# OpenDriveLab/ThinkTwice

Hardware: AMD Instinct MI355X
Metric: frames/sec forward (4-cam+LiDAR, thinktwice.py cfg) (higher is better)
Workload: dtype bf16x3h; 1 GPU; forward_inference thinktwice.py cfg: 8 frames x (2 sweeps x 4 cams x 448x896 + 65536-pt LiDAR), ResNet50+PAFPN+DepthNet+UNet+LSS splat, LidarNet, fusion, 5-stage decoder; parallelism=replicas x1 (no data-path collective), launch=eager launches, 3 batches in flight on alternating streams, batches_in_flight=3

## Files before the change

### include/thinktwice_hip.h

```cpp
#ifndef THINKTWICE_HIP_H
#define THINKTWICE_HIP_H

#include <stddef.h>
#include <stdint.h>

#ifdef __cplusplus
extern "C" {
#endif

#define TT_F32 0
#define TT_BF16 1
#define TT_F16 2

#define TT_ACT_NONE 0
#define TT_ACT_RELU 1
#define TT_ACT_SIGMOID 2
#define TT_ACT_GELU 3
#define TT_ACT_SOFTPLUS 4
#define TT_ACT_SOFTPLUS_CLAMP 5

const char* tt_last_error(void);
const char* tt_conv_last_kernel(void);
int tt_conv_set_trace(void* stamps_or_null);
int tt_version(void);

int tt_voxel_pool_fwd(int batch_size, int num_points, int num_channels,
                      int num_voxel_x, int num_voxel_y, int num_voxel_z,
                      const int32_t* geom_xyz, const float* input_features,
                      float* output_features, int32_t* pos_memo, void* stream);

long long tt_voxel_pool_workspace_bytes(int batch_size, int num_points, int num_channels,
                                        int num_voxel_x, int num_voxel_y);
int tt_voxel_pool_fwd_ws(int batch_size, int num_points, int num_channels,
                         int num_voxel_x, int num_voxel_y, int num_voxel_z,
                         const int32_t* geom_xyz, const float* input_features,
                         float* output_features, int32_t* pos_memo,
                         void* workspace, long long workspace_bytes, void* stream);

long long tt_voxel_pool_plan_bytes(int batch_size, int num_points, int num_voxel_x, int num_voxel_y);
long long tt_voxel_pool_plan_workspace_bytes(int batch_size, int num_points);
int tt_voxel_pool_plan_build(int batch_size, int num_points, int num_voxel_x, int num_voxel_y, int num_voxel_z,
                             const int32_t* geom_xyz, void* workspace, long long workspace_bytes, void* plan,
                             long long plan_bytes, void* stream);
long long tt_voxel_pool_planned_workspace_bytes(int batch_size, int num_points, int num_channels, int num_voxel_x,
                                                int num_voxel_y);
int tt_voxel_pool_fwd_planned(int batch_size, int num_points, int num_channels, int num_voxel_x, int num_voxel_y,
                              const void* plan, const float* input_features, float* output_features, void* workspace,
                              long long workspace_bytes, void* stream);

int tt_voxel_pool_bwd(int batch_size, int num_points, int num_channels,
                      int num_voxel_x, int num_voxel_y,
                      const int32_t* pos_memo, const float* grad_out_bhwc,
                      float* grad_in, void* stream);

int tt_frustum_voxel_index(int batch_size, int num_cams, int D, int fH, int fW,
                           const float* frustum, const float* mats,
                           const float* voxel_lo, const float* voxel_size,
                           int32_t* geom_xyz, float* geom_f32_or_null,
                           void* stream);

int tt_lift_splat_fwd(int batch_size, int num_cams, int D, int fH, int fW, int C,
                      int num_voxel_x, int num_voxel_y, int num_voxel_z,
                      const void* depth_logits, const void* context, int dtype,
                      const int32_t* geom_xyz, float* out, int out_cstride,
                      int out_coff, int rot_flip, void* stream);

long long tt_lift_splat_workspace_bytes(int batch_size, int num_cams, int D, int fH, int fW, int C,
                                        int num_voxel_x, int num_voxel_y);
int tt_lift_splat_fwd_ws(int batch_size, int num_cams, int D, int fH, int fW, int C,
                         int num_voxel_x, int num_voxel_y, int num_voxel_z,
                         const void* depth_logits, const void* context, int dtype,
                         const int32_t* geom_xyz, float* out, int out_cstride,
                         int out_coff, int rot_flip, void* ws, long long ws_bytes, void* stream);

typedef struct tt_conv_desc {
    const void* in;   int N, H, W, Cin, in_cstride, in_coff;
    long long in_nstride;
    const void* weight; int Cout, KH, KW, stride, pad, dil;
    void* out; int OH, OW, out_cstride, out_coff;
    long long out_nstride;
    int pixel_shuffle2;
    const float* scale; const float* shift;
    const float* shift_n; int shift_n_mod;
    const void* res1; int res1_cstride, res1_coff;
    const void* res2; int res2_cstride, res2_coff;
    int act;
    int dtype;
    int out_dtype;
    const int* gather_idx;
    const int* m_dev;
    float* splitk_ws;
    const void* weight_x3;
    const int* row_perm;
    const unsigned* row_mask;
    int splitk_slices;
    int in_pair, out_pair;
    const void* weight_h2;
    float* out2; int out2_cstride, out2_coff;
    int res1_up_h, res1_up_w;
    int res1_f32;
    int in_up2;
} tt_conv_desc;

int tt_conv2d_fwd(const tt_conv_desc* d, void* stream);
int tt_conv2d_splitk_slices(const tt_conv_desc* d);
int tt_conv2d_plan(const tt_conv_desc* d, char* label, int label_bytes);

int tt_seg_feedback_chain(const float* x, long long R, int x_stride, int K1, const float* w1, const float* scale1,
                          const float* shift1, int act1, const float* w2, const void* w2_x3, int N2, const float* scale2,
                          const float* shift2, int act2, float* out, int out_stride, int out_coff, void* stream);

typedef struct tt_chain_stage {
    const void* w; const float* bias;
    int K, Kp, N, act, in_sel;
    const float* res; int res_stride, res_coff;
    const float* side; const float* side_w; int side_stride, side_k;
    float* out; int out_stride, out_coff;
} tt_chain_stage;
int tt_mlp_chain(const float* x, long long R, int x_stride, int nstages, const tt_chain_stage* stages, int n_split,
                 void* stream);
long long tt_mlp_chain_wide_workspace_bytes(long long R, int nstages, const tt_chain_stage* stages);
int tt_mlp_chain_wide(const float* x, long long R, int x_stride, int nstages, const tt_chain_stage* stages, int n_groups,
                      void* workspace, long long workspace_bytes, void* stream);
int tt_mlp_chain_wide_max_workgroups(void);
int tt_mlp_chain_wide_faults(void);
int tt_device_faults(void);
int tt_clear_device_faults(void);
int tt_mlp_chain_wide_set_max_spin(int polls);
int tt_mlp_chain_wide_set_trace(void* stamps_or_null);

long long tt_dec_gru_scratch_floats(int B);
int tt_dec_gru(int B, const float* inp6, const float* state, float* fut, float* scratch, const void* const* w0,
               const float* const* wx, const float* const* b0, const void* const* w2, const float* const* b2,
               const void* wd0, const float* bd0, const void* wd2, const float* bd2, void* stream);
long long tt_dec_flatten_scratch_floats(int maps);
int tt_dec_flatten(int maps, const float* in, float* out, float* mids_or_null, float* scratch, const void* const* w,
                   const float* const* b, const float* bn_scale, const float* bn_shift, void* stream);
int tt_dec_set_trace(void* stamps_or_null);
long long tt_dec_bev_update_scratch_floats(int B);
int tt_dec_bev_update(int B, const float* bev, const float* G, float* out, long long out_bstride, float* out2,
                      long long out2_bstride, float* scratch, const void* w0, const float* b0, const void* const* w2,
                      const float* b2, void* stream);

int tt_nchw_to_nhwc_pad(const float* in, void* out, int N, int C, int H, int W, int Cp,
                        int out_dtype, void* stream);
int tt_nchw_to_nhwc_border(const float* in, void* out, int N, int C, int H, int W, int Cp, int Hp, int Wp,
                           int top, int left, int out_dtype, void* stream);
int tt_nhwc_to_nchw(const void* in, float* out, int N, int C, int H, int W, int cstride, int coff,
                    int in_dtype, void* stream);
int tt_maxpool3x3s2(const void* in, void* out, int N, int H, int W, int C, int dtype, void* stream);
int tt_upsample_nearest_add(void* dst, const void* src, int N, int H, int W, int C, int h, int w,
                            int dtype, void* stream);
int tt_bilinear_up2(const void* in, void* out, int N, int H, int W, int C, int dtype, void* stream);
int tt_bilinear_up2_pair(const float* in, float* out, int N, int H, int W, int C, void* stream);
int tt_spatial_pool(const void* in, float* out, int N, int HW, int C, int cstride, int coff, int mode,
                    int dtype, void* stream);
int tt_channel_gate(const void* x, const float* gate, const void* res, void* out, int N, int HW, int C,
                    int gate_act, int out_act, int dtype, void* stream);
int tt_affine_rows(const void* x, const float* scale, const float* shift, void* out, long long R, int C,
                   int x_stride, int out_stride, int act, int dtype, void* stream);
int tt_layernorm_rows(const void* x, const float* gamma, const float* beta, void* out, long long R,
                      int D, int x_stride, int out_stride, float eps, int dtype, void* stream);
int tt_copy_nhwc(const void* in, void* out, int N, int H, int W, int C, int in_cstride, int in_coff,
                 int out_cstride, int out_coff, int rot_flip, int in_dtype, int out_dtype, void* stream);
int tt_broadcast_rows(const void* v, void* out, int N, int HW, int C, int v_stride, int out_cstride,
                      int out_coff, int dtype, void* stream);
int tt_ew(const void* a, const void* b, const void* g, void* out, long long R, int C, int a_stride,
          int a_coff, int b_stride, int b_coff, int g_stride, int g_coff, int o_stride, int o_coff,
          int op, int act, int dtype, void* stream);
int tt_concat_rows(float* out, long long R, int out_stride, int nseg, const float* const* srcs, const int* strides,
                   const int* widths, const int* coffs, const int* divs, const int* mods, void* stream);

int tt_deform_im2col3x3(const void* x, const float* offsets, void* cols, int N, int H, int W, int C,
                        int off_cstride, int pad, int dtype, void* stream);

int tt_look_project_pack(int B, const float* wp, const float* lidar2img, const float* ida_mat,
                         float img_h, float img_w, float* ref_packed, int* query_of_slot,
                         int* count, int* max_len, void* stream);
int tt_look_gather_query(int B, const int* query_of_slot, const float* ref_packed, const float* wp,
                         const float* ctrl_softplus, const float* temporal_embedding,
                         const float* static_embedding, const float* measurement_feat,
                         const float* flattened_feat, const void* const* level_maps,
                         const int* level_hw, int maps_dtype, float* out, int row_stride, void* stream);
int tt_msda_sample(int B, const void* value, int value_dtype, const float* offsets, const float* logits,
                   const float* ref_packed, const int* level_hw, float* out, void* stream);
int tt_msda_sample_strided(int B, const void* value, int value_dtype, int value_cstride, int value_coff,
                           const float* offsets, const float* logits, const float* ref_packed, const int* level_hw,
                           float* out, void* stream);
int tt_sca_reduce(int B, const float* x, const int* max_len, float* out, void* stream);
// ... 316 lines not shown
```

### thinktwice_amd/csrc/conv_igemm.hip

```cpp
#include <stdlib.h>

#include "conv_common.h"

namespace tt {

template <typename T, int BM, int BN, int WAVES_M, int WAVES_N, bool GATHER, int KX = 1>
__global__ __launch_bounds__(256) void conv_igemm_kernel(const ConvArgs p) {
    constexpr int VEC = Elem<T>::kVec;
    constexpr int BKB = ((sizeof(T) == 4) ? 64 : 128) * KX;
    constexpr int BK = BKB / (int)sizeof(T);
    constexpr int VPR = BKB / 16;
    constexpr int ROWB = BKB + 16;
    constexpr int NVA = (BM * VPR + 255) / 256;
    constexpr int NVB = (BN * VPR + 255) / 256;
    constexpr int WTM = BM / WAVES_M, WTN = BN / WAVES_N;
    constexpr int TM = WTM / 32, TN = WTN / 32;
    static_assert(WAVES_M * WAVES_N == 4, "4 waves");

    extern __shared__ __attribute__((aligned(16))) unsigned char smem[];
    const int nbuf = (p.K > BK) ? 2 : 1;
    unsigned char* sA = smem;
    unsigned char* sB = smem + nbuf * BM * ROWB;

    const int tid = threadIdx.x;
    const int lane = tid & 63;
    const int wave = tid >> 6;
    const int wm = wave / WAVES_N, wn = wave % WAVES_N;

    const int tile_n = blockIdx.x % p.tiles_n;
    const int tile_m = blockIdx.x / p.tiles_n;
    const int m0 = tile_m * BM, n0 = tile_n * BN;
    int Mlim = p.M;
    if (p.m_dev) {
        const int md = *p.m_dev;
        Mlim = md < Mlim ? md : Mlim;
    }
    if (m0 >= Mlim) return;

    const T* __restrict__ in = reinterpret_cast<const T*>(p.in);
    const T* __restrict__ wgt = reinterpret_cast<const T*>(p.weight);

    int a_row[NVA], a_vc[NVA], a_h0[NVA], a_w0[NVA];
    long long a_base[NVA];
    bool a_ok[NVA];
#pragma unroll
    for (int i = 0; i < NVA; ++i) {
        const int idx = tid + 256 * i;
        a_row[i] = idx / VPR;
        a_vc[i] = idx % VPR;
        const int m = m0 + a_row[i];
        a_ok[i] = (m < Mlim) && (idx < BM * VPR);
        const int mm = a_ok[i] ? m : 0;
        if (GATHER) {
            a_h0[i] = 0;
            a_w0[i] = 0;
            a_base[i] = (long long)mm * (p.KH * p.KW);
        } else {
            const int n = mm / (p.OH * p.OW);
            const int r = mm - n * (p.OH * p.OW);
            const int oh = r / p.OW, ow = r - oh * p.OW;
            a_h0[i] = oh * p.stride - p.pad;
            a_w0[i] = ow * p.stride - p.pad;
            a_base[i] = (long long)n * p.in_nstride + p.in_coff;
        }
    }
    int b_row[NVB], b_vc[NVB];
    bool b_ok[NVB];
#pragma unroll
    for (int i = 0; i < NVB; ++i) {
        const int idx = tid + 256 * i;
        b_row[i] = idx / VPR;
        b_vc[i] = idx % VPR;
        b_ok[i] = ((n0 + b_row[i]) < p.Cout) && (idx < BN * VPR);
    }

    int jn[NVA];
#pragma unroll
    for (int i = 0; i < NVA; ++i) jn[i] = -1;
    const int nk_all = (p.K + BK - 1) / BK;
    int kt0 = 0, nk = nk_all;
    if (p.splits > 1) {
        const int per = (nk_all + p.splits - 1) / p.splits;
        kt0 = blockIdx.y * per;
        nk = min(nk_all, kt0 + per);
        if (kt0 >= nk) return;
// ... 290 lines not shown
    ConvChoice c;
    if (const int r = conv2d_prepare(d, a, f)) return r;
    if (const int r = conv_choose(a, f, &c)) return r;
    hipStream_t st = (hipStream_t)stream;
    const bool pair = d->in_pair || d->out_pair;
    const char* what = "tt_conv2d_fwd";
    int r;
    if (c.x3) a.weight = d->weight_x3;
    switch (c.family) {
        case CONV_H2:
        case CONV_H2_PIPE:
            a.weight = d->weight_h2;
            what = "tt_conv2d_fwd(h2)";
            r = launch_conv_h2(c, a, st);
            break;
        case CONV_SMALL:
            what = "tt_conv2d_fwd(small)";
            r = launch_conv_small(a, d->dtype, st);
            break;
        case CONV_SP_RUNS_L2:
            what = "tt_conv2d_fwd(sp l2)";
            r = launch_sp_conv_l2(c, a, st);
            break;
        case CONV_SP_RUNS:
            what = "tt_conv2d_fwd(glds x3)";
            r = launch_sp_conv_runs(c, a, st);
            break;
        case CONV_X3_PIPE:
        case CONV_X3_RUN3:
            what = pair ? "tt_conv2d_fwd(glds x3, pair)" : "tt_conv2d_fwd(glds x3)";
            r = launch_conv_x3_pipe(c, a, st);
            break;
        case CONV_X3_UP2:
            what = "tt_conv2d_fwd(x3 up2)";
            r = launch_conv_x3_up2(c, a, st);
            break;
        case CONV_X3_PATCH:
            what = "tt_conv2d_fwd(x3 patch, pair)";
            r = launch_conv_x3_patch(c, a, st);
            break;
        case CONV_GLDS:
            what = !c.x3 ? "tt_conv2d_fwd(glds)" : c.splits > 1 ? "tt_conv2d_fwd(glds x3 split-K)" : pair ? "tt_conv2d_fwd(glds x3, pair)" : "tt_conv2d_fwd(glds x3)";
            if (c.splits > 1) a.ws_slices = c.slices;
            r = launch_conv_glds(c, a, d->dtype, st);
            break;
        default:
            a.row_perm = nullptr;
            a.row_mask = nullptr;
            r = launch_conv_igemm(c, a, d->dtype, st);
            break;
    }
    if (r < 0) return r;
    conv_label(c, d->dtype, g_conv_kernel, sizeof(g_conv_kernel));
    if (c.main_rows > 0) {
        ConvArgs t = a;
        t.m_begin = c.main_rows * 256;
        if (launch_conv_glds(conv_tail_choice(c), t, d->dtype, st) < 0) return -1;
    }
    if (c.splits > 1) launch_splitk_finalize(a, d->dtype, st);
    return check_launch(what);
}

extern "C" int tt_conv2d_splitk_slices(const tt_conv_desc* d) {
    ConvArgs a;
    ConvFacts f;
    ConvChoice c;
    if (conv2d_prepare(d, a, f)) return 0;
    if (d->in_pair || d->out_pair || d->in_up2 || d->weight_h2 || d->res1_up_w > 0) return 0;
    f.assume_ws = true;
    if (conv_choose(a, f, &c)) return 0;
    return c.splits > 1 ? c.slices : 0;
}

extern "C" int tt_conv2d_plan(const tt_conv_desc* d, char* label, int label_bytes) {
    ConvArgs a;
    ConvFacts f;
    ConvChoice c;
    if (const int r = conv2d_prepare(d, a, f)) return r;
    if (const int r = conv_choose(a, f, &c)) return r;
    TT_REQUIRE(label && label_bytes > 0, "tt_conv2d_plan: no room for the label");
    conv_label(c, d->dtype, label, (size_t)label_bytes);
    return 0;
}
```

### thinktwice_amd/csrc/conv_igemm_glds.hip

```cpp
#include "conv_lds_dma.h"

namespace tt {

#ifndef TT_GLDS_DEBUG
#define TT_GLDS_DEBUG 0
#endif

template <typename T, int BN, int WAVES_M, int WAVES_N, int BKB, int STAGES = 3, bool GATHER = false, bool X3 = false, bool APAIR = false>
__global__ __launch_bounds__(WAVES_M * WAVES_N * 64,
                             ((256 / WAVES_M / 32) * (BN / WAVES_N / 32) >= 16)  ? 1
                             : ((256 / WAVES_M / 32) * (BN / WAVES_N / 32) >= 8) ? 2
                             : (WAVES_M * WAVES_N == 16 || BKB == 64)            ? 4
                                                                                 : 2)
void conv_igemm_glds_kernel(const ConvArgs p, const void* zero_page,
                                                              int tiles_m, int tiles_n) {
#if defined(__HIP_DEVICE_COMPILE__)
    constexpr int BM = 256;
    constexpr int VEC = Elem<T>::kVec;
    constexpr int BK = BKB / (int)sizeof(T);
    constexpr int CPR = BKB / 16;
    constexpr bool ASYM = STAGES == 23;
    constexpr int SA = ASYM ? 3 : STAGES, SB = ASYM ? 2 : STAGES;
    static_assert(STAGES == 2 || STAGES == 3 || ASYM, "2 or 3 LDS stages, or 23 = 3 activation + 2 weight stages");
    static_assert(!GATHER || STAGES == 2, "gather mode is written for the 2-stage pipeline");
// ... 64 lines not shown
    const T* b_ptr[NIB];
#pragma unroll
    for (int j = 0; j < NIB; ++j) {
        const int g = ((wave + NW * j) % NB_INSTR) * 64 + lane;
        const int row = g / CPR, pos = g % CPR;
        b_c[j] = (pos ^ swz<BKB>(row)) * VEC;
        b_ok[j] = (n0 + row) < p.Cout;
        b_base[j] = (long long)(n0 + row) * p.K;
        b_ptr[j] = wgt + b_base[j] + b_c[j];
    }

    int nk = (p.K + BK - 1) / BK;

    int g_cur[NIA];
    int g_t = 0;
    const int cin_shift = 31 - __clz(p.Cin), cin_mask = p.Cin - 1;
    constexpr int TPTMAX = 4;
    const bool planned = GATHER && p.row_mask != nullptr;
    unsigned umask = 0;
    if (planned) {
        unsigned* uw = reinterpret_cast<unsigned*>(smem);
        if (tid == 0) *uw = 0u;
        __syncthreads();
        if (tid < BM && m0 + tid < Mlim) atomicOr(uw, p.row_mask[m0 + tid]);
        __syncthreads();
        umask = *uw;
        __syncthreads();
        umask = __builtin_amdgcn_readfirstlane(umask);
        const int nt = __popc(umask);
        nk = p.Cin >= BK ? nt * (p.Cin / BK) : (nt * p.Cin + BK - 1) / BK;
    }
    struct TapWalk {
        unsigned rem;
        int sub, cur;
    };
    TapWalk wf{umask, 0, -1}, wi{umask, 0, -1};
    auto next_taps = [&](TapWalk& w, int (&tp)[TPTMAX]) {
        if (p.Cin >= BK) {
            if (w.sub == 0) {
                w.cur = w.rem ? __builtin_ctz(w.rem) : -1;
                w.rem &= w.rem - 1;
            }
            tp[0] = w.cur;
            if (++w.sub == p.Cin / BK) w.sub = 0;
        } else {
            const int tpt = BK >> cin_shift;
#pragma unroll
            for (int i = 0; i < TPTMAX; ++i) {
                tp[i] = -1;
                if (i < tpt && w.rem) {
                    tp[i] = __builtin_ctz(w.rem);
                    w.rem &= w.rem - 1;
                }
            }
        }
    };
    auto pick = [&](const int (&tp)[TPTMAX], int slot) {
        int t = tp[0];
#pragma unroll
        for (int i = 1; i < TPTMAX; ++i) t = (slot == i) ? tp[i] : t;
        return t;
    };
    auto fetch_rulebook = [&]() {
        if (planned) {
            int tp[TPTMAX];
            next_taps(wf, tp);
#pragma unroll
            for (int j = 0; j < NIA; ++j) {
                const int t = p.Cin >= BK ? tp[0] : pick(tp, a_c[j] >> cin_shift);
                g_cur[j] = (a_ok[j] && t >= 0) ? p.gather[a_base[j] + t] : -1;
            }
            ++g_t;
            return;
        }
#pragma unroll
        for (int j = 0; j < NIA; ++j) {
            const int k = g_t * BK + a_c[j];
            g_cur[j] = (a_ok[j] && k < p.K) ? p.gather[a_base[j] + (k >> cin_shift)] : -1;
        }
        ++g_t;
    };
    const int wave_s = __builtin_amdgcn_readfirstlane(wave);
    const unsigned lds_dma_base = (unsigned)(uintptr_t)(__attribute__((address_space(3))) unsigned char*)smem;
    KWalk wa{0, 0, 0}, wb{0, 0, 0};
    if (!GATHER && p.splits > 1) {
        const int per = (nk + p.splits - 1) / p.splits;
        const int kt0 = (int)blockIdx.y * per;
        int kt1 = kt0 + per;
        kt1 = kt1 < nk ? kt1 : nk;
        const int taps = p.KH * p.KW;
        const int chunk = kt0 / taps, tap = kt0 - chunk * taps;
        wa.ci = wb.ci = chunk * BK;
        wa.kh = wb.kh = tap / p.KW;
        wa.kw = wb.kw = tap - (tap / p.KW) * p.KW;
        nk = kt1 > kt0 ? kt1 - kt0 : 0;
    }
    auto issue_a = [&](int kt) {
        const unsigned st = lds_dma_base + (unsigned)off_a(kt);
        const int kh = wa.kh, kw = wa.kw, ci = wa.ci;
        const int k0 = kt * BK;
        const int tap = kh * p.KW + kw;
        const long long tap_off = ((long long)(kh * p.dil) * p.W + kw * p.dil) * p.in_cstride + ci;
        advance<BK>(wa, p);
        const bool dbg_skip_a = TT_GLDS_DEBUG && p.act == 98 && kt > 0;
#pragma unroll
        for (int j = 0; j < NIA; ++j) {
            if (dbg_skip_a) break;
            const T* src;
            if (GATHER) {
                const int gi = g_cur[j];
                const int kl = k0 + a_c[j];
                src = gi >= 0 ? in + (long long)gi * p.in_cstride + p.in_coff + (kl & cin_mask) : zp;
            } else {
                src = ((a_mask[j] >> tap) & 1u) ? a_ptr[j] + tap_off : zp;
            }
            dma_piece(src, st + (unsigned)(wave_s + NW * j) * 1024u);
        }
    };
    auto issue_b = [&](int kt) {
        const unsigned st = lds_dma_base + (unsigned)off_b(kt);
        const int k0 = GATHER ? kt * BK
                              : (wb.kh * p.KW + wb.kw) * p.Cin + wb.ci;
        advance<BK>(wb, p);
        const bool dbg_skip_b = TT_GLDS_DEBUG && p.act == 97 && kt > 0;
        int tpi[TPTMAX];
        if (planned) next_taps(wi, tpi);
#pragma unroll
        for (int j = 0; j < NIB; ++j) {
            if (dbg_skip_b) break;
            bool ok = b_ok[j] && (!GATHER || (k0 + b_c[j] < p.K));
            const T* src = ok ? b_ptr[j] + k0 : zp;
            if (planned) {
                const int t = p.Cin >= BK ? tpi[0] : pick(tpi, b_c[j] >> cin_shift);
                ok = b_ok[j] && t >= 0;
                src = ok ? b_ptr[j] - b_c[j] + (long long)t * p.Cin + ((k0 + b_c[j]) & cin_mask) : zp;
            }
            dma_piece(src, st + (unsigned)((wave_s + NW * j) % NB_INSTR) * 1024u);
        }
    };
    auto issue_tile = [&](int kt) {
        issue_a(kt);
        issue_b(kt);
    };
    auto issue_ahead = [&](int kt) {
        if (ASYM) {
            if (kt + 1 < nk) issue_b(kt + 1);
            if (kt + 2 < nk) issue_a(kt + 2);
        } else if (kt + STAGES - 1 < nk) {
            issue_tile(kt + STAGES - 1);
        }
    };

    auto a_begin = [&](int kt, bool on) { return dma_begin_a<BK>(p, wa, lds_dma_base + (unsigned)off_a(kt), on); };
    auto b_begin = [&](int kt, bool on) { return dma_begin_b<BK, 1>(p, wb, lds_dma_base + (unsigned)off_b(kt), on); };
    auto a_emit = [&](const DmaCtx& c, int j) { dma_emit_a(c, a_ptr[j], a_mask[j], zp, wave_s + NW * j); };
    auto b_emit = [&](const DmaCtx& c, int j) { dma_emit_b(c, b_ptr[j], b_ok[j], zp, (wave_s + NW * j) % NB_INSTR); };

    f32x16 acc[TM][TN];
    zero_acc(acc);

    if (GATHER && nk > 0) fetch_rulebook();
    if (nk > 0) issue_tile(0);
    if (GATHER && nk > 1) fetch_rulebook();
    if (STAGES == 3 && nk > 1) issue_tile(1);
    if (ASYM && nk > 1) issue_a(1);

    const unsigned lds_base = (unsigned)(uintptr_t)(__attribute__((address_space(3))) unsigned char*)smem;
    unsigned fa_off[TM], fb_off[TN], fa_s[TM], fb_s[TN];
    const unsigned hi = lane >> 5;
#pragma unroll
    for (int i = 0; i < TM; ++i) {
        const int row = wm * WTM + i * 32 + (lane & 31);
        fa_off[i] = row * BKB;
        fa_s[i] = swz<BKB>(row);
    }
#pragma unroll
    for (int j = 0; j < TN; ++j) {
        const int row = wn * WTN + j * 32 + (lane & 31);
        fb_off[j] = BM * BKB + row * BKB;
        fb_s[j] = swz<BKB>(row);
    }
    constexpr int NKC_ = X3 ? BKB / 64 : BKB / 32;
    const bool spread = BN == 256;
    unsigned fa_pre[NKC_][TM], fb_pre[NKC_][TN];
#pragma unroll
    for (int kc = 0; kc < NKC_; ++kc) {
        const unsigned ca = X3 ? (APAIR ? 4u * kc + hi : 4u * kc + 2u * hi) : 2u * kc + hi;
        const unsigned cb = X3 ? 4u * kc + hi : 2u * kc + hi;
#pragma unroll
        for (int i = 0; i < TM; ++i) fa_pre[kc][i] = fa_off[i] + ((ca ^ fa_s[i]) << 4);
#pragma unroll
        for (int j = 0; j < TN; ++j) fb_pre[kc][j] = fb_off[j] + ((cb ^ fb_s[j]) << 4);
    }

    for (int kt = 0; kt < nk; ++kt) {
        if (ASYM && kt + 1 < nk) wait_vmcnt<NIA>();
        else if (STAGES == 3 && kt + 1 < nk) wait_vmcnt<LPT>();
        else wait_vmcnt<0>();
        asm volatile("s_barrier" ::: "memory");
        if (tr && kt == 0) tr[1] = (long long)wall_clock64();

        const unsigned sbase_a = lds_base + (unsigned)off_a(kt);
        const unsigned sbase_b = lds_base + (unsigned)(off_b(kt) - A_BYTES);
        const unsigned sbase = sbase_a;
        if constexpr (X3) {
            constexpr int NS = NKC_ * TN;
            u32x4 ra0[TM], ra1[TM], bh[2], bl[2];
            uint4 ah[2][TM], al[2][TM];
            auto split_frag = [&](int i, uint4& hi_out, uint4& lo_out) {
                asm volatile("" : "+v"(ra0[i]));
                asm volatile("" : "+v"(ra1[i]));
                if (APAIR || (TT_GLDS_DEBUG && p.act == 96)) {
                    hi_out = __builtin_bit_cast(uint4, ra0[i]);
                    lo_out = __builtin_bit_cast(uint4, ra1[i]);
                    return;
                }
                split8(ra0[i], ra1[i], hi_out, lo_out);
            };
#pragma unroll
            for (int i = 0; i < TM; ++i) {
                ra0[i] = lds_read(sbase + fa_pre[0][i]);
                ra1[i] = lds_read(sbase + (fa_pre[0][i] ^ (APAIR ? 32u : 16u)));
            }
            bh[0] = lds_read(sbase_b + fb_pre[0][0]);
            bl[0] = lds_read(sbase_b + (fb_pre[0][0] ^ 32u));
            constexpr bool SPREAD = !GATHER;
            constexpr int PER = (NIA + NIB + NS - 1) / NS;
            DmaCtx ca{0u, 0, 0, false}, cb{0u, 0, 0, false};
            if constexpr (SPREAD) {
                if (spread) {
                    if (ASYM) {
                        cb = b_begin(kt + 1, kt + 1 < nk);
                        ca = a_begin(kt + 2, kt + 2 < nk);
                    } else {
                        ca = a_begin(kt + STAGES - 1, kt + STAGES - 1 < nk);
                        cb = b_begin(kt + STAGES - 1, kt + STAGES - 1 < nk);
                    }
// ... 164 lines not shown
```

### thinktwice_amd/csrc/conv_lds_dma.h

```cpp
#pragma once
#include "conv_common.h"

namespace tt {

typedef __attribute__((address_space(3))) void* lds_ptr_t;
typedef unsigned u32x4 __attribute__((ext_vector_type(4)));

__device__ __forceinline__ u32x4 lds_read(unsigned addr) {
    u32x4 v;
    asm volatile("ds_read_b128 %0, %1" : "=v"(v) : "v"(addr) : "memory");
    return v;
}

template <int N>
__device__ __forceinline__ void wait_vmcnt() {
    static_assert(N >= 0 && N <= 63, "vmcnt is a 6-bit count");
    asm volatile("s_waitcnt vmcnt(%0)" ::"n"(N) : "memory");
}

template <typename E>
__device__ __forceinline__ void dma_piece(const E* src, unsigned lds) {
    __builtin_amdgcn_global_load_lds(src, (lds_ptr_t)(uintptr_t)lds, 16, 0, 0);
}

template <int ROWB>
__device__ __forceinline__ int swz(int row) {
    static_assert(ROWB == 64 || ROWB == 128 || ROWB == 256, "64 B, 128 B or 256 B rows");
    return ROWB == 64 ? (row >> 2) & 3 : ROWB == 128 ? (row >> 1) & 7 : row & 15;
}

template <int ROWB>
__device__ __forceinline__ unsigned frag_off(int row, unsigned chunk) {
    return row * ROWB + ((chunk ^ swz<ROWB>(row)) << 4);
}

__device__ __forceinline__ int xcd_tile(int nblk) {
    const int b = blockIdx.x, xcd = b & 7, q = nblk >> 3, r = nblk & 7;
    return (xcd < r ? xcd * (q + 1) : r * (q + 1) + (xcd - r) * q) + (b >> 3);
}

struct RowWindow {
    int n, h0, w0;
};
__device__ __forceinline__ RowWindow row_window(const ConvArgs& p, int m) {
    const int n = m / (p.OH * p.OW);
    const int r = m - n * (p.OH * p.OW);
    const int oh = r / p.OW, ow = r - oh * p.OW;
    return RowWindow{n, oh * p.stride - p.pad, ow * p.stride - p.pad};
}
__device__ __forceinline__ unsigned tap_mask(const ConvArgs& p, int h0, int w0) {
    unsigned mk = 0;
    int tbit = 0;
    for (int kh = 0; kh < p.KH; ++kh) {
        const int ih = h0 + kh * p.dil;
        for (int kw = 0; kw < p.KW; ++kw, ++tbit) {
            const int iw = w0 + kw * p.dil;
            if (ih >= 0 && ih < p.H && iw >= 0 && iw < p.W) mk |= 1u << tbit;
        }
    }
    return mk;
}
template <int ROWB, typename E>
__device__ __forceinline__ void dense_slot(const ConvArgs& p, const E* in, int g, int m0, int Mlim, const E*& ptr, unsigned& mask) {
    constexpr int CPR = ROWB / 16, VEC = 16 / (int)sizeof(E);
    const int row = g / CPR, pos = g % CPR;
    const int c = (pos ^ swz<ROWB>(row)) * VEC;
    const int m = m0 + row;
    const bool ok = m < Mlim;
    const RowWindow w = row_window(p, ok ? m : 0);
    ptr = in + (long long)w.n * p.in_nstride + p.in_coff + ((long long)w.h0 * p.W + w.w0) * p.in_cstride + c;
    mask = ok ? tap_mask(p, w.h0, w.w0) : 0u;
}

struct KWalk {
    int kh, kw, ci;
};
template <int BK>
__device__ __forceinline__ void advance(KWalk& w, const ConvArgs& p) {
    if (++w.kw == p.KW) {
        w.kw = 0;
        if (++w.kh == p.KH) {
            w.kh = 0;
            w.ci += BK;
        }
    }
}
struct DmaCtx {
    unsigned st;
    int tap;
    long long off;
    bool on;
};
template <int BK>
__device__ __forceinline__ DmaCtx dma_begin_a(const ConvArgs& p, KWalk& w, unsigned st, bool on) {
    DmaCtx c{0u, 0, 0, on};
    if (!on) return c;
    c.st = st;
    c.tap = w.kh * p.KW + w.kw;
    c.off = ((long long)(w.kh * p.dil) * p.W + w.kw * p.dil) * p.in_cstride + w.ci;
    advance<BK>(w, p);
    return c;
}
template <int BK, int WROW>
__device__ __forceinline__ DmaCtx dma_begin_b(const ConvArgs& p, KWalk& w, unsigned st, bool on) {
    DmaCtx c{0u, 0, 0, on};
    if (!on) return c;
    c.st = st;
    c.off = (long long)WROW * ((long long)(w.kh * p.KW + w.kw) * p.Cin + w.ci);
    advance<BK>(w, p);
    return c;
}
template <typename E>
__device__ __forceinline__ void dma_emit_a(const DmaCtx& c, const E* ptr, unsigned mask, const E* zp, int piece) {
    dma_piece(((mask >> c.tap) & 1u) ? ptr + c.off : zp, c.st + (unsigned)piece * 1024u);
}
template <typename E>
__device__ __forceinline__ void dma_emit_b(const DmaCtx& c, const E* ptr, bool ok, const E* zp, int piece) {
    dma_piece(ok ? ptr + c.off : zp, c.st + (unsigned)piece * 1024u);
}

template <typename K, typename... Extra>
static int launch_lds_dma(K kern, dim3 grid, dim3 block, size_t lds, size_t lds_max, const char* who, ConvArgs& a, hipStream_t st,
                          int tiles_m, int tiles_n, int splits, Extra... extra) {
    const void* zp = zero_page(who);
    if (!zp || lds_opt_in(reinterpret_cast<const void*>(kern), lds_max, who)) return -1;
    a.tiles_n = tiles_n;
    a.splits = splits;
    if (splits <= 1) a.ws = nullptr;
    hipLaunchKernelGGL(kern, grid, block, lds, st, a, zp, tiles_m, tiles_n, extra...);
    return 1;
}

}
```

### thinktwice_amd/csrc/conv_x3_pipe.hip

```cpp
#include "conv_lds_dma.h"

namespace tt {

#ifndef TT_PIPE_DEBUG
#define TT_PIPE_DEBUG 0
#endif

template <int WAVES_M, int WAVES_N, int BN = 256, bool APAIR = false>
__global__ __launch_bounds__(256, 1) void conv_x3_pipe_kernel(const ConvArgs p, const void* zero_page, int tiles_m,
                                                             int tiles_n) {
#if defined(__HIP_DEVICE_COMPILE__)
    constexpr int BM = 256, BKB = 128, BK = 32;
    constexpr int NW = WAVES_M * WAVES_N;
    constexpr int WTM = BM / WAVES_M, WTN = BN / WAVES_N;
    constexpr int TM = WTM / 32, TN = WTN / 32;
    static_assert(NW == 4 && (TM * TN == 16 || TM * TN == 8) && TN % TM == 0,
                  "four waves of 128 x 128 (2 x 2) or 64 x 256 (4 x 1) on a 256 x 256 tile; of 64 x 128 (4 x 1) on a 256 x 128 tile");
    constexpr int A_BYTES = BM * BKB, B_BYTES = BN * BKB;
    constexpr int NIA = BM * 8 / 64 / NW, NIB = BN * 8 / 64 / NW;
    constexpr int MG = 3 * TM;
    constexpr int NGR = TN / TM;
    constexpr int WIN = NGR * MG;
    constexpr int DPA = NIA / TN, DPB = NIB / TN;
    static_assert(NIA % TN == 0 && NIB % TN == 0 && DPA >= 1 && DPA <= 2 && DPB >= 1 && DPB <= 2, "one or two DMA pieces per group");
    static_assert(WIN >= 12, "a row-block window needs 12 gaps for the barrier, the fragment reads and the split");

    extern __shared__ __attribute__((aligned(16))) unsigned char smem[];
    const int tid = threadIdx.x, lane = tid & 63, wave = tid >> 6;
    const int wm = wave / WAVES_N, wn = wave % WAVES_N;
    const int Mlim = p.M;

    const int nblk = tiles_m * tiles_n;
    if ((int)blockIdx.x >= nblk) return;
    const int L = xcd_tile(nblk);
    const int tile_n = L % tiles_n, tile_m = L / tiles_n;
    const int m0 = p.m_begin + tile_m * BM, n0 = tile_n * BN;
    if (m0 >= Mlim) return;

    const float* __restrict__ in = reinterpret_cast<const float*>(p.in);
    const float* __restrict__ wgt = reinterpret_cast<const float*>(p.weight);
    const float* zp = reinterpret_cast<const float*>(zero_page);

    const float* a_ptr[NIA];
    unsigned a_mask[NIA];
#pragma unroll
    for (int j = 0; j < NIA; ++j) dense_slot<BKB>(p, in, (wave + NW * j) * 64 + lane, m0, Mlim, a_ptr[j], a_mask[j]);
    const float* b_ptr0;
    {
        const int g = wave * 64 + lane;
        const int row = g >> 3, pos = g & 7;
        b_ptr0 = wgt + (long long)(n0 + row) * p.K + (pos ^ swz<BKB>(row)) * 4;
    }
    const long long b_jstride = (long long)(NW * 8) * p.K;

    const int nk = p.K / BK;
    const int wave_s = __builtin_amdgcn_readfirstlane(wave);
    const unsigned lds_base = (unsigned)(uintptr_t)(__attribute__((address_space(3))) unsigned char*)smem;
    const unsigned ldsA = lds_base, ldsB = lds_base + 3u * A_BYTES;

    const int ntaps = p.KH * p.KW;
    const long long a_d1 = (long long)p.dil * p.in_cstride;
    const long long a_d2 = ((long long)p.dil * p.W - (long long)(p.KW - 1) * p.dil) * p.in_cstride;
    const long long a_d3 = BK - ((long long)(p.KH - 1) * p.dil * p.W + (long long)(p.KW - 1) * p.dil) * p.in_cstride;
    const long long a_e2 = a_d2 - a_d1, a_e3 = a_d3 - a_d2;
    const long long b_d1 = p.Cin;
    const long long b_e2 = (BK - (long long)(ntaps - 1) * p.Cin) - b_d1;
    int a_kw = 0, a_tap = 0, a_rem = nk;
    long long a_off = 0;
    unsigned a_st = ldsA;
    int b_tap = 0, b_rem = nk, b_w = 0;
    long long b_off = 0;
    unsigned b_st = ldsB;
    long long a_d = 0;
    auto a_walk1 = [&]() {
        const int kw1 = a_kw + 1;
        const bool w1 = kw1 == p.KW;
        a_kw = w1 ? 0 : kw1;
        a_d = a_d1 + (w1 ? a_e2 : 0ll);
    };
    auto a_walk2 = [&]() {
        const int tp1 = a_tap + 1;
        const bool w2 = tp1 == ntaps;
        a_tap = w2 ? 0 : tp1;
        a_off += a_d + (w2 ? a_e3 : 0ll);
    };
    auto a_walk3 = [&]() {
        a_rem -= 1;
        a_st = a_st == ldsA + 2u * A_BYTES ? ldsA : a_st + A_BYTES;
    };
    auto b_walk1 = [&]() {
        const int tp1 = b_tap + 1;
        const bool adv = b_rem > 1;
        b_w = tp1 == ntaps;
        b_off += (adv ? b_d1 : 0ll) + ((adv && b_w) ? b_e2 : 0ll);
        b_tap = adv ? (b_w ? 0 : tp1) : b_tap;
    };
    auto b_walk2 = [&]() {
        b_rem -= 1;
        b_st = b_st == ldsB ? ldsB + B_BYTES : ldsB;
    };
    auto a_emit = [&](int j) {
        const int tapbit = a_rem > 0 ? a_tap : 31;
        const float* src = ((a_mask[j] >> tapbit) & 1u) ? a_ptr[j] + a_off : zp;
        dma_piece(src, a_st + (unsigned)(wave_s + NW * j) * 1024u);
    };
    auto b_emit = [&](int j) {
        const float* src = b_ptr0 + b_off + (long long)j * b_jstride;
        dma_piece(src, b_st + (unsigned)(wave_s + NW * j) * 1024u);
    };

    f32x16 acc[TM][TN];
    zero_acc(acc);

    const unsigned hi = lane >> 5;
    unsigned fa_pre[2][TM], fb_pre[2][TN];
#pragma unroll
    for (int kc = 0; kc < 2; ++kc) {
#pragma unroll
        for (int i = 0; i < TM; ++i) fa_pre[kc][i] = frag_off<BKB>(wm * WTM + i * 32 + (lane & 31), 4u * kc + (APAIR ? hi : 2u * hi));
#pragma unroll
        for (int j = 0; j < TN; ++j) fb_pre[kc][j] = frag_off<BKB>(wn * WTN + j * 32 + (lane & 31), 4u * kc + hi);
    }
#if TT_PIPE_DEBUG & 4
#define TT_MFMA(c, a, b) asm volatile("" : "+a"(c) : "v"(a), "v"(b))
#else
#define TT_MFMA(c, a, b) asm volatile("v_mfma_f32_32x32x16_bf16 %0, %1, %2, %0" : "+a"(c) : "v"(a), "v"(b))
#endif

    u32x4 ah[2][TM], al[2][TM];
    u32x4 bh[TN], bl[TN];
    u32x4 ra0, ra1;

    {
#pragma unroll
        for (int t = 0; t < 2; ++t) {
#pragma unroll
            for (int j = 0; j < NIA; ++j) a_emit(j);
            a_walk1(); a_walk2(); a_walk3();
#pragma unroll
            for (int j = 0; j < NIB; ++j) b_emit(j);
            b_walk1(); b_walk2();
        }
        wait_vmcnt<NIA + NIB>();
        asm volatile("s_barrier" ::: "memory");
#pragma unroll
        for (int i = 0; i < TM; ++i) {
// ... 544 lines not shown
```

Before: 113.1 frames/s.

## Skip dead kernel-row taps per output tile in padded x3 conv kernels

Adds a per-tile analysis of which kernel taps can touch valid input pixels given the tile's output rows and padding, then trims the K loop to the live kernel-row range in the x3 pipe kernel and the x3 LDS-DMA igemm kernel when split-K is off. Pointers and validity masks are shifted past the dead leading rows and the K walk uses the reduced row count. This avoids loading zero-page data and running MMA work for taps that only hit padding at image borders. The cost is some extra per-block index arithmetic, and tiles inside the image still run every tap.

```diff
diff --git a/include/thinktwice_hip.h b/include/thinktwice_hip.h
--- a/include/thinktwice_hip.h
+++ b/include/thinktwice_hip.h
@@ -105,6 +105,7 @@
 int tt_conv2d_fwd(const tt_conv_desc* d, void* stream);
 int tt_conv2d_splitk_slices(const tt_conv_desc* d);
 int tt_conv2d_plan(const tt_conv_desc* d, char* label, int label_bytes);
+int tt_conv2d_tap_range(const tt_conv_desc* d, long long m0, int rows, int* lo, int* hi);
 
 int tt_seg_feedback_chain(const float* x, long long R, int x_stride, int K1, const float* w1, const float* scale1,
                           const float* shift1, int act1, const float* w2, const void* w2_x3, int N2, const float* scale2,
diff --git a/thinktwice_amd/csrc/conv_igemm.hip b/thinktwice_amd/csrc/conv_igemm.hip
--- a/thinktwice_amd/csrc/conv_igemm.hip
+++ b/thinktwice_amd/csrc/conv_igemm.hip
@@ -1,6 +1,7 @@
 #include <stdlib.h>
 
 #include "conv_common.h"
+#include "conv_tap_range.h"
 
 namespace tt {
 
@@ -457,3 +458,17 @@
     conv_label(c, d->dtype, label, (size_t)label_bytes);
     return 0;
 }
+
+extern "C" int tt_conv2d_tap_range(const tt_conv_desc* d, long long m0, int rows, int* lo, int* hi) {
+    ConvArgs a;
+    ConvFacts f;
+    if (const int r = conv2d_prepare(d, a, f)) return r;
+    TT_REQUIRE(lo && hi, "tt_conv2d_tap_range: null pointer");
+    TT_REQUIRE(!d->gather_idx, "tt_conv2d_tap_range: a gathered layer has no tap geometry (its rulebook names the taps)");
+    TT_REQUIRE(m0 >= 0 && m0 < a.M && rows > 0, "tt_conv2d_tap_range: rows [%lld, %lld + %d) outside the layer's %d output rows", m0, m0,
+               rows, a.M);
+    const TapRange r = conv_tap_range(a, (int)m0, rows);
+    *lo = r.lo;
+    *hi = r.hi;
+    return 0;
+}
diff --git a/thinktwice_amd/csrc/conv_igemm_glds.hip b/thinktwice_amd/csrc/conv_igemm_glds.hip
--- a/thinktwice_amd/csrc/conv_igemm_glds.hip
+++ b/thinktwice_amd/csrc/conv_igemm_glds.hip
@@ -170,7 +170,25 @@
     };
     const int wave_s = __builtin_amdgcn_readfirstlane(wave);
     const unsigned lds_dma_base = (unsigned)(uintptr_t)(__attribute__((address_space(3))) unsigned char*)smem;
-    KWalk wa{0, 0, 0}, wb{0, 0, 0};
+    constexpr bool RANGE = X3 && !GATHER;
+    KWalk wa{0, 0, 0, p.KH}, wb = wa;
+    if constexpr (RANGE) {
+        if (p.splits <= 1) {
+            const TapRange live = conv_tap_range<false>(p, m0, BM);
+            const int kh_lo = __builtin_amdgcn_readfirstlane(live.lo) / p.KW;
+            const int kh_hi = (__builtin_amdgcn_readfirstlane(live.hi) + p.KW - 1) / p.KW;
+            const long long skip_a = (long long)kh_lo * p.dil * p.W * p.in_cstride, skip_b = (long long)kh_lo * p.KW * p.Cin;
+#pragma unroll
+            for (int j = 0; j < NIA; ++j) {
+                a_ptr[j] += skip_a;
+                a_mask[j] >>= kh_lo * p.KW;
+            }
+#pragma unroll
+            for (int j = 0; j < NIB; ++j) b_ptr[j] += skip_b;
+            wa.nkh = wb.nkh = kh_hi - kh_lo;
+            nk = (p.Cin / BK) * (kh_hi - kh_lo) * p.KW;
+        }
+    }
     if (!GATHER && p.splits > 1) {
         const int per = (nk + p.splits - 1) / p.splits;
         const int kt0 = (int)blockIdx.y * per;
@@ -189,7 +207,7 @@
         const int k0 = kt * BK;
         const int tap = kh * p.KW + kw;
         const long long tap_off = ((long long)(kh * p.dil) * p.W + kw * p.dil) * p.in_cstride + ci;
-        advance<BK>(wa, p);
+        advance<BK, RANGE>(wa, p);
         const bool dbg_skip_a = TT_GLDS_DEBUG && p.act == 98 && kt > 0;
 #pragma unroll
         for (int j = 0; j < NIA; ++j) {
@@ -209,7 +227,7 @@
         const unsigned st = lds_dma_base + (unsigned)off_b(kt);
         const int k0 = GATHER ? kt * BK
                               : (wb.kh * p.KW + wb.kw) * p.Cin + wb.ci;
-        advance<BK>(wb, p);
+        advance<BK, RANGE>(wb, p);
         const bool dbg_skip_b = TT_GLDS_DEBUG && p.act == 97 && kt > 0;
         int tpi[TPTMAX];
         if (planned) next_taps(wi, tpi);
@@ -239,8 +257,8 @@
         }
     };
 
-    auto a_begin = [&](int kt, bool on) { return dma_begin_a<BK>(p, wa, lds_dma_base + (unsigned)off_a(kt), on); };
-    auto b_begin = [&](int kt, bool on) { return dma_begin_b<BK, 1>(p, wb, lds_dma_base + (unsigned)off_b(kt), on); };
+    auto a_begin = [&](int kt, bool on) { return dma_begin_a<BK, RANGE>(p, wa, lds_dma_base + (unsigned)off_a(kt), on); };
+    auto b_begin = [&](int kt, bool on) { return dma_begin_b<BK, 1, RANGE>(p, wb, lds_dma_base + (unsigned)off_b(kt), on); };
     auto a_emit = [&](const DmaCtx& c, int j) { dma_emit_a(c, a_ptr[j], a_mask[j], zp, wave_s + NW * j); };
     auto b_emit = [&](const DmaCtx& c, int j) { dma_emit_b(c, b_ptr[j], b_ok[j], zp, (wave_s + NW * j) % NB_INSTR); };
 
diff --git a/thinktwice_amd/csrc/conv_lds_dma.h b/thinktwice_amd/csrc/conv_lds_dma.h
--- a/thinktwice_amd/csrc/conv_lds_dma.h
+++ b/thinktwice_amd/csrc/conv_lds_dma.h
@@ -1,5 +1,6 @@
 #pragma once
 #include "conv_common.h"
+#include "conv_tap_range.h"
 
 namespace tt {
 
@@ -74,12 +75,13 @@
 
 struct KWalk {
     int kh, kw, ci;
+    int nkh;
 };
-template <int BK>
+template <int BK, bool RANGE = false>
 __device__ __forceinline__ void advance(KWalk& w, const ConvArgs& p) {
     if (++w.kw == p.KW) {
         w.kw = 0;
-        if (++w.kh == p.KH) {
+        if (++w.kh == (RANGE ? w.nkh : p.KH)) {
             w.kh = 0;
             w.ci += BK;
         }
@@ -91,23 +93,23 @@
     long long off;
     bool on;
 };
-template <int BK>
+template <int BK, bool RANGE = false>
 __device__ __forceinline__ DmaCtx dma_begin_a(const ConvArgs& p, KWalk& w, unsigned st, bool on) {
     DmaCtx c{0u, 0, 0, on};
     if (!on) return c;
     c.st = st;
     c.tap = w.kh * p.KW + w.kw;
     c.off = ((long long)(w.kh * p.dil) * p.W + w.kw * p.dil) * p.in_cstride + w.ci;
-    advance<BK>(w, p);
+    advance<BK, RANGE>(w, p);
     return c;
 }
-template <int BK, int WROW>
+template <int BK, int WROW, bool RANGE = false>
 __device__ __forceinline__ DmaCtx dma_begin_b(const ConvArgs& p, KWalk& w, unsigned st, bool on) {
     DmaCtx c{0u, 0, 0, on};
     if (!on) return c;
     c.st = st;
     c.off = (long long)WROW * ((long long)(w.kh * p.KW + w.kw) * p.Cin + w.ci);
-    advance<BK>(w, p);
+    advance<BK, RANGE>(w, p);
     return c;
 }
 template <typename E>
diff --git a/thinktwice_amd/csrc/conv_tap_range.h b/thinktwice_amd/csrc/conv_tap_range.h
--- /dev/null
+++ b/thinktwice_amd/csrc/conv_tap_range.h
@@ -0,0 +1,70 @@
+#pragma once
+#include "conv_choose.h"
+
+namespace tt {
+
+struct TapRange {
+    int lo, hi;
+};
+
+__host__ __device__ inline void tap_axis_live(int o0, int o1, int stride, int c, int size, int& a, int& b) {
+    if (stride == 1) {
+        a = o0 > -c ? o0 : -c;
+        b = o1 < size - 1 - c ? o1 : size - 1 - c;
+    } else {
+        const bool any = o1 * stride + c >= 0 && o0 * stride + c < size;
+        a = o0;
+        b = any ? o1 : o0 - 1;
+    }
+}
+
+template <bool KW_EXACT>
+__host__ __device__ inline void tap_range_segment(const ConvArgs& p, int r0, int r1, int& lo, int& hi) {
+    const int oh0 = r0 / p.OW, oh1 = r1 / p.OW;
+    for (int kh = 0; kh < p.KH; ++kh) {
+        int a, b;
+        tap_axis_live(oh0, oh1, p.stride, kh * p.dil - p.pad, p.H, a, b);
+        if (a > b) continue;
+        int kw_lo = 0, kw_hi = p.KW - 1;
+        if (KW_EXACT && a == b) {
+            const int w0 = r0 > a * p.OW ? r0 - a * p.OW : 0, w1 = r1 < a * p.OW + p.OW - 1 ? r1 - a * p.OW : p.OW - 1;
+            kw_lo = p.KW;
+            kw_hi = -1;
+            for (int kw = 0; kw < p.KW; ++kw) {
+                int wa, wb;
+                tap_axis_live(w0, w1, p.stride, kw * p.dil - p.pad, p.W, wa, wb);
+                if (wa <= wb) {
+                    kw_lo = kw < kw_lo ? kw : kw_lo;
+                    kw_hi = kw;
+                }
+            }
+            if (kw_lo > kw_hi) continue;
+        }
+        const int first = kh * p.KW + kw_lo, last = kh * p.KW + kw_hi;
+        lo = first < lo ? first : lo;
+        hi = last + 1 > hi ? last + 1 : hi;
+    }
+}
+
+template <bool KW_EXACT = true>
+__host__ __device__ inline TapRange conv_tap_range(const ConvArgs& p, int m0, int rows) {
+    const int ntaps = p.KH * p.KW;
+    const TapRange all{0, ntaps};
+    const int m1 = (rows < p.M - m0 ? m0 + rows : p.M) - 1;
+    if (ntaps == 1 || p.pad == 0 || p.gather || m0 < 0 || m1 < m0) return all;
+    const int ohw = p.OH * p.OW;
+    const int n0 = m0 / ohw, r0 = m0 - n0 * ohw;
+    int lo = ntaps, hi = 0;
+    if (m1 - m0 < ohw - r0) {
+        tap_range_segment<KW_EXACT>(p, r0, r0 + (m1 - m0), lo, hi);
+    } else {
+        const int n1 = m1 / ohw, r1 = m1 - n1 * ohw;
+        tap_range_segment<KW_EXACT>(p, r0, ohw - 1, lo, hi);
+        tap_range_segment<KW_EXACT>(p, 0, r1, lo, hi);
+        if (n1 > n0 + 1) tap_range_segment<KW_EXACT>(p, 0, ohw - 1, lo, hi);
+    }
+    if (lo >= hi) return TapRange{0, 1};
+    return TapRange{lo, hi};
+}
+
+}
diff --git a/thinktwice_amd/csrc/conv_x3_pipe.hip b/thinktwice_amd/csrc/conv_x3_pipe.hip
--- a/thinktwice_amd/csrc/conv_x3_pipe.hip
+++ b/thinktwice_amd/csrc/conv_x3_pipe.hip
@@ -1,4 +1,5 @@
 #include "conv_lds_dma.h"
+#include "conv_tap_range.h"
 
 namespace tt {
 
@@ -53,15 +54,29 @@
     }
     const long long b_jstride = (long long)(NW * 8) * p.K;
 
-    const int nk = p.K / BK;
+    const TapRange live = conv_tap_range<false>(p, m0, BM);
+    const int kh_lo = __builtin_amdgcn_readfirstlane(live.lo) / p.KW;
+    const int kh_hi = (__builtin_amdgcn_readfirstlane(live.hi) + p.KW - 1) / p.KW;
+    const int t_lo = kh_lo * p.KW;
+    const int ntaps = (kh_hi - kh_lo) * p.KW;
+    {
+        const long long skip = (long long)kh_lo * p.dil * p.W * p.in_cstride;
+#pragma unroll
+        for (int j = 0; j < NIA; ++j) {
+            a_ptr[j] += skip;
+            a_mask[j] >>= t_lo;
+        }
+        b_ptr0 += (long long)t_lo * p.Cin;
+    }
+    const int nk = (p.Cin / BK) * ntaps;
     const int wave_s = __builtin_amdgcn_readfirstlane(wave);
     const unsigned lds_base = (unsigned)(uintptr_t)(__attribute__((address_space(3))) unsigned char*)smem;
     const unsigned ldsA = lds_base, ldsB = lds_base + 3u * A_BYTES;
 
-    const int ntaps = p.KH * p.KW;
+    const int nkh = kh_hi - kh_lo;
     const long long a_d1 = (long long)p.dil * p.in_cstride;
     const long long a_d2 = ((long long)p.dil * p.W - (long long)(p.KW - 1) * p.dil) * p.in_cstride;
-    const long long a_d3 = BK - ((long long)(p.KH - 1) * p.dil * p.W + (long long)(p.KW - 1) * p.dil) * p.in_cstride;
+    const long long a_d3 = BK - ((long long)(nkh - 1) * p.dil * p.W + (long long)(p.KW - 1) * p.dil) * p.in_cstride;
     const long long a_e2 = a_d2 - a_d1, a_e3 = a_d3 - a_d2;
     const long long b_d1 = p.Cin;
     const long long b_e2 = (BK - (long long)(ntaps - 1) * p.Cin) - b_d1;
```

Result: no change. 113.4 frames/s, median of 6 (+0.3%).
